# zfkuang/PaletteNeRF

Hardware: AMD Instinct MI355X
Metric: rendered_samples_per_sec (higher is better)
Workload: dtype f32 (field: f16x3 split products, fp32 accumulate); 1 GPU; configs[1]: NeRF-synthetic lego geometry (scene S0), -m nerf inference, 800x800, 1 view(s)/step, camera moving (one pose of the path per step); march_mode=native, fused_field=True, field_precision=f16x3, half_tables=False, ray_order=tile8, frames_in_flight=1, gathered_floats_per_ray=0, rccl_ranks=1, parallelism=single GPU

## Files before the change

### palettenerf_amd/csrc/frame.hip

```cpp
#include "pnr_common.hpp"
#include "march_core.hpp"
#include "grid_core.hpp"
#include "field_core.hpp"
#include "frame_plan.hpp"
#include <hip/hip_ext.h>
#include <vector>
#include <stdlib.h>

uint64_t pnr_internal_edit_device_bytes();
int pnr_internal_edit_upload(const pnr_palette_edit* edit, void* dst, hipStream_t s);
int pnr_internal_palette_field_forward(const pnr_palette_field_args* a, pnr_stream_t stream, int waves12);

#ifndef PNR_FRAME_LEVEL_PAIRS
#define PNR_FRAME_LEVEL_PAIRS 1
#endif
#ifndef PNR_FRAME_LEVEL_PAIRS_PAL
#define PNR_FRAME_LEVEL_PAIRS_PAL 0
#endif
namespace pnr {

struct FrameCtl {
    int32_t n_alive, n_step, step, done;
    int32_t iterations, pad0;
    unsigned long long rendered;
// ... 110 lines not shown
                                                                    float* __restrict__ depth, float* __restrict__ image, float* __restrict__ aux,
                                                                    FrameFinish fin) {
    if (fin.ctl && !fin.ctl->done) return;
    const uint32_t i = (blockIdx.x * kRayBlock + threadIdx.x) / LANES, q = threadIdx.x % LANES;
    if (i >= N) return;
    const uint32_t r = order ? (uint32_t)order[i] : i;
    if (q == 0) {
        const float d = sdepth[i];
        if (order) ws[r] = sws[i];
        if (fin.depth_raw) fin.depth_raw[r] = d;
        depth[r] = (fin.on & 2) ? finish_depth(fin, d, r) : d;
    }
    if (q < 3) { const float v = simage[(size_t)i * 3 + q]; image[(size_t)r * 3 + q] = (fin.on & 1) ? finish_channel(fin, v, sws[i], r, q) : v; }
    if (saux) {
        if (q * 4 < aux_stride) {
            float4 v = *reinterpret_cast<const float4*>(saux + (size_t)i * aux_stride + q * 4);
            if (q == 0 && (fin.on & 4)) {
                const float w = sws[i];
                v.x = finish_channel(fin, v.x, w, r, 0); v.y = finish_channel(fin, v.y, w, r, 1); v.z = finish_channel(fin, v.z, w, r, 2);
            }
            *reinterpret_cast<float4*>(aux + (size_t)r * aux_stride + q * 4) = v;
        }
    } else if (aux && (fin.on & 4) && q < 3) {
        aux[(size_t)r * aux_stride + q] = finish_channel(fin, aux[(size_t)r * aux_stride + q], sws[i], r, q);
    }
}

#ifdef PNR_MARCH_STATS
__device__ unsigned long long g_march_stats[8];
__device__ unsigned int g_march_max[64];
__device__ unsigned int g_march_hist[2][32];
__device__ unsigned int g_march_kinds[64][8];
#endif
__device__ __forceinline__ uint32_t shfl_xor_fresh(uint32_t v, int off) {
    int lane = (int)__builtin_amdgcn_mbcnt_hi(~0u, __builtin_amdgcn_mbcnt_lo(~0u, 0u));
    asm volatile("" : "+v"(lane));
    return (uint32_t)__builtin_amdgcn_ds_bpermute((lane ^ off) << 2, (int)v);
}
__device__ __forceinline__ unsigned long long shfl_xor_fresh(unsigned long long v, int off) {
    return ((unsigned long long)shfl_xor_fresh((uint32_t)(v >> 32), off) << 32) | shfl_xor_fresh((uint32_t)v, off);
}
__device__ __forceinline__ unsigned long long block_sum_u64(unsigned long long v, unsigned long long* sh ) {
    for (int off = PNR_WAVE / 2; off > 0; off >>= 1) v += shfl_xor_fresh(v, off);
    __syncthreads();
    if ((threadIdx.x & (PNR_WAVE - 1)) == 0) sh[threadIdx.x / PNR_WAVE] = v;
    __syncthreads();
    unsigned long long t = 0;
    for (int wv = 0; wv < (int)(kRayBlock / PNR_WAVE); wv++) t += sh[wv];
    return t;
}


#ifdef PNR_MARCH_TIMING
constexpr int kTimingWaves = 8192;
__device__ unsigned long long g_march_timing[kTimingWaves * 8];
__device__ int g_march_timing_iter = 3;
#define PNR_STAMP(k) do { if (timing && (threadIdx.x & 63) == 0) g_march_timing[(size_t)twave * 8 + (k)] = wall_clock64(); } while (0)
#else
#define PNR_STAMP(k) do { } while (0)
#endif
#ifndef PNR_MARCH_WAVES
#define PNR_MARCH_WAVES 4
#endif
#ifndef PNR_MARCH2_JUMPS
#define PNR_MARCH2_JUMPS true
#endif
#ifndef PNR_MARCH_WAVES_Q
#define PNR_MARCH_WAVES_Q 5
#endif
template <bool MIP, bool POW2, int MODE>
__global__ void __launch_bounds__(kRayBlock) __attribute__((amdgpu_waves_per_eu(MODE == 2 ? PNR_MARCH_WAVES_Q : PNR_MARCH_WAVES))) k_frame_march(const FrameCtl* __restrict__ prev, FrameCtl* __restrict__ cur, const int32_t* __restrict__ alive_prev,
                                                           int32_t* __restrict__ rays_alive, const int32_t* __restrict__ counts ,
                                                           int32_t* __restrict__ counts_cur ,
                                                           int32_t* __restrict__ scratch_rw, uint32_t N, uint32_t max_steps,
// ... 80 lines not shown
    const uint32_t* mip_lds = nullptr;
    if (mip_fast) {
        asm volatile("s_waitcnt vmcnt(0)" ::: "memory");
        __syncthreads();
        mip_lds = mip_smem;
    } else {
        mip_lds = stage_mip(mip, MIP ? p.mip_words : 0);
    }
    PNR_STAMP(2);
    uint32_t emitted = 0;
    uint32_t base = (uint32_t)(sums & 0xffffffffull), summed_to = blockIdx.x;
    for (uint32_t chunk = blockIdx.x; chunk < nchunks; chunk += gridDim.x) {
        if (threadIdx.x == 0) counts_cur[chunk] = 0;
        int index = index0;
        if (chunk != blockIdx.x) {
            unsigned long long pre = 0;
            for (uint32_t j = summed_to + threadIdx.x; j < chunk; j += kRayBlock) pre += (unsigned long long)counts[j];
            base += (uint32_t)block_sum_u64(pre, red);
            summed_to = chunk;
            const uint32_t slot = chunk * kRayBlock + threadIdx.x;
            index = slot < n_prev ? alive_prev[slot] : -1;
        }
        const int keep = index >= 0 ? 1 : 0;
        const unsigned long long alive_mask = __ballot(keep);
        if (lane == 0) csum[wave] = __popcll(alive_mask);
        __syncthreads();
        int woff = 0;
        for (int wv = 0; wv < wave; wv++) woff += csum[wv];
        __syncthreads();
        PNR_STAMP(3);
        uint32_t n = 0, step = 0;
        float t = 0.0f, far = -FLT_MAX, last_t = 0.0f;
        RayCtx c = {};
        if (keep) {
            n = base + (uint32_t)woff + (uint32_t)__popcll(alive_mask & ((1ull << lane) - 1ull));
            rays_alive[n] = index;
            ctx_init(c, rays_o + (size_t)index * 3, rays_d + (size_t)index * 3, p, grid, mip_lds);
            t = rays_t[index];
            const BoxHit bh = clip_to_box(c, fars[index]);
            far = bh.far;
            const float noise = (noises && prev->iterations == -1) ? noises[index] : 0.0f;
            t = fmaf(clampf(t * c.dt_gamma, c.dt_min, c.dt_max), noise, t);
            last_t = t;
            t = skip_to_box<MIP && POW2>(c, bh, t);
        }
        PNR_STAMP(4);
#ifdef PNR_MARCH_TIMING
        uint32_t my_probes = 0;
#endif
#ifdef PNR_MARCH_STATS
        unsigned long long probes = 0, empties = 0;
        unsigned int kinds[8] = {0, 0, 0, 0, 0, 0, 0, 0};
#endif
        bool active = keep && t < far;
        [[maybe_unused]] bool queued = false;
        [[maybe_unused]] uint32_t step_queued = 0;
        for (uint32_t round = 0;; round++) {
            const unsigned long long am = __ballot(active);
            if (am == 0ull) break;
            if constexpr (MODE == 1) { if (p.coop && __popcll(am) <= kCoopRays) break; }
            if constexpr (MODE == 2) {
                const bool give_up = active && round - step >= budget;
                const unsigned long long gm = __ballot(give_up);
                if (gm != 0ull) {
                    int32_t* qctr = qctr_all + ((prev->iterations + 1) & 1) * kQueueCtrs;
                    const int leader = __ffsll((long long)gm) - 1;
                    int slot0 = 0;
                    if (lane == leader) slot0 = atomicAdd(&qctr[0], __popcll(gm));
                    slot0 = __builtin_amdgcn_readlane(slot0, leader);
                    if (give_up) {
                        StragglerRec r;
                        r.n = (int32_t)n; r.index = index; r.step = (int32_t)step; r.t = t; r.last_t = last_t; r.far = far; r.pad0 = 0; r.pad1 = 0;
                        qrecs[(uint32_t)slot0 + (uint32_t)__popcll(gm & ((1ull << lane) - 1ull))] = r;
                        queued = true; step_queued = step; active = false;
                    }
                    if (gm == am) break;
                }
            }
// ... 663 lines not shown
    w.alive[1] = reinterpret_cast<int32_t*>(take(n * 4));
    w.rays_t = reinterpret_cast<float*>(take(n * 4));
    w.xyzs = reinterpret_cast<float*>(take(n * 12));
    w.dirs = reinterpret_cast<float*>(take(n * 12));
    w.deltas = reinterpret_cast<float*>(take(n * 8));
    w.enc = reinterpret_cast<float*>(take(n * 16 * 2 * 4));
    w.sigmas = reinterpret_cast<float*>(take(n * 4));
    w.rgbs = reinterpret_cast<float*>(take(n * 12));
    w.scratch = reinterpret_cast<int32_t*>(take((kHdr + 2 * (n / kRayBlock + 2)) * 4));
    w.partials[0] = reinterpret_cast<int32_t*>(take((kMaxMarchBlocks + kHostedBlocks) * 4));
    w.partials[1] = reinterpret_cast<int32_t*>(take((kMaxMarchBlocks + kHostedBlocks) * 4));
    w.enc_pal = w.enc_clip = w.aux = nullptr;
    w.edit = nullptr;
    if (aux_stride) {
        w.edit = take(pnr_internal_edit_device_bytes());
        w.enc_pal = reinterpret_cast<float*>(take(n * 16 * 2 * 4));
        if (with_clip) w.enc_clip = reinterpret_cast<float*>(take(n * 16 * 2 * 4));
        w.aux = reinterpret_cast<float*>(take(n * aux_stride * 4));
    }
    w.s_o = reinterpret_cast<float*>(take(n * 12)); w.s_d = reinterpret_cast<float*>(take(n * 12));
    w.s_noise = reinterpret_cast<float*>(take(n * 4)); w.s_far = reinterpret_cast<float*>(take(n * 4));
    w.s_ws = reinterpret_cast<float*>(take(n * 4)); w.s_depth = reinterpret_cast<float*>(take(n * 4));
    w.s_image = reinterpret_cast<float*>(take(n * 12));
    w.s_aux = aux_stride ? reinterpret_cast<float*>(take(n * aux_stride * 4)) : nullptr;
    w.hosted = reinterpret_cast<HostedConst*>(take(sizeof(HostedConst)));
    w.qctr = reinterpret_cast<int32_t*>(take(2 * kQueueCtrs * 4));
    w.qrecs = reinterpret_cast<StragglerRec*>(take(n * sizeof(StragglerRec)));
    w.rowflag = reinterpret_cast<uint8_t*>(take(n));
    w.bytes = off;
    return w;
}

struct FrameOpts {
    int aux_fusion, composite_fusion, hosted_tail, dynamic_tiles, march_budget, march_budget0, march_blocks, iteration_margin, block_skip, coop_march, palette_waves12;
};
static FrameOpts frame_opts_now() {
    return FrameOpts{g_opt_aux_fusion, g_opt_composite_fusion, g_opt_hosted_tail, g_opt_dynamic_tiles, g_opt_march_budget, g_opt_march_budget0, g_opt_march_blocks,
                     g_opt_iteration_margin, g_opt_block_skip, g_opt_coop_march, g_opt_palette_waves12};
}

using UnsortKernel = decltype(&k_frame_unsort_outputs<4>);
using MarchKernel = decltype(&k_frame_march<true, true, 1>);
using GridKernel = decltype(&k_frame_grid);
using FieldKernel = decltype(&k_frame_field<0, false>);

struct FramePlan {
    pnr_stream_t stream; const void* workspace;
    uint32_t N, max_steps, aux_stride, n_enc, march_lds;
    float T_thresh, density_scale, enc_scale;
    FrameWorkspace w;
    const float *in_o, *in_d, *in_far, *noise_p;
    float *out_ws, *out_depth, *out_image, *out_aux;
    const int32_t* ray_order;
    float *ray_ws, *ray_depth, *ray_image, *ray_aux;
    const uint8_t* bitfield; const uint32_t* mip; const float* packed_weights;
    bool with_clip, half_tables, hosted, use_mip, pow2, pal_composite_fused, timing, has_edit;
    int aux_fused;
    int composite_fused;
    MarchParams mp;
    GridArgs ga;
    pnr_palette_field_args pf;
    pnr_palette_edit edit;
    FrameFinish fin;
    FrameOpts opt;
    MarchKernel march, march_budgeted;
    GridKernel lookup; uint32_t lookup_y, lookup_z;
    FieldKernel field;
    uint64_t* stats; float* kernel_ms;
};
struct FrameProgress { int iter = 0; uint32_t alive_ub = 0, chunk = 0, looks = 0, prev_partials = 0; size_t ev_used = 0; };
struct PerDevice {
// ... 82 lines not shown
    ga.enc[0] = w.enc; ga.enc[1] = w.enc_pal; ga.enc[2] = w.enc_clip;
    p.lookup_y = 16; p.lookup_z = 1;
    if (p.half_tables && pal && p.with_clip) { p.lookup = k_frame_grid_h3; ga.table[0] = pal->embeddings_triple; }
    else if (p.half_tables && pal) { p.lookup = k_frame_grid_h2; ga.table[0] = pal->embeddings_pair; }
    else if (p.half_tables) { p.lookup = k_frame_grid_h1; ga.table[0] = a->embeddings; }
    else if (pal && p.with_clip && pal->embeddings_triple) { p.lookup = k_frame_grid_triple; ga.table[0] = pal->embeddings_triple; }
    else if (pal && !p.with_clip && pal->embeddings_pair) { p.lookup = k_frame_grid_pair; ga.table[0] = pal->embeddings_pair; p.lookup_y = PNR_FRAME_LEVEL_PAIRS_PAL ? 8 : 16; }
    else {
        p.lookup = k_frame_grid; p.lookup_y = PNR_FRAME_LEVEL_PAIRS == 2 ? 4 : (PNR_FRAME_LEVEL_PAIRS ? 8 : 16); p.lookup_z = p.n_enc;
        ga.table[0] = a->embeddings; ga.table[1] = pal ? pal->embeddings_palette : nullptr; ga.table[2] = p.with_clip ? pal->embeddings_clip : nullptr;
    }

    if (pal) {
        pnr_palette_field_args& pf = p.pf;
        pf.enc = w.enc; pf.enc_palette = w.enc_pal; pf.enc_clip = w.enc_clip; pf.level_stride = p.N; pf.dirs = w.dirs; pf.deltas = w.deltas;
        pf.packed = a->packed_weights; pf.num_basis = pal->num_basis;
        pf.clip_dim = pal->clip_dim; pf.pred_clip = pal->pred_clip; pf.density_scale = a->density_scale; pf.offsets_weight = pal->offsets_weight;
        pf.view_dep_weight = pal->view_dep_weight; pf.aux_stride = p.aux_stride; pf.sigmas = w.sigmas; pf.rgbs = w.rgbs; pf.aux = w.aux;
        pf.precision = a->field_precision; pf.xyzs = w.xyzs;
        for (int k = 0; k < 3; k++) pf.enc_scale[k] = a->enc_scale[k];
        pf.overflow_flag = a->watch_overflow ? w.scratch + 1 : nullptr;
        pf.tile_counter = opt.dynamic_tiles ? w.scratch + 2 : nullptr;
        if (p.aux_fused) { pf.weights_sum = p.out_ws; pf.aux_map = p.out_aux; pf.T_thresh = a->T_thresh; }
        if (p.pal_composite_fused) { pf.rays_t = w.rays_t; pf.weights_sum_rw = p.out_ws; pf.depth = p.out_depth; pf.image = p.out_image; }
        if (pal->edit && pal->edit->mode != 0) { p.has_edit = true; p.edit = *pal->edit; pf.edit_device = w.edit; }
    } else {
        p.enc_scale = a->enc_scale[0] > 0.0f ? a->enc_scale[0] : 1.0f;
        p.field = frame_field_kernel(a->field_precision, a->watch_overflow);
    }

    p.use_mip = a->mip && (a->H % 4) == 0 && pnr_occupancy_mip_bytes(a->C, a->H) <= 64 * 1024;
    p.pow2 = is_pow2f(a->bound) && (a->H & (a->H - 1)) == 0;
    p.mp = make_march_params(a->bound, a->dt_gamma, a->max_steps, a->C, a->H, p.use_mip);
    p.mp.block_skip = opt.block_skip ? 1u : 0u; p.mp.coop = opt.coop_march ? 1u : 0u;
    p.march_lds = p.mp.mip_words ? (2 * p.mp.mip_words + 8) * 4 : 0;
    p.hosted = opt.hosted_tail && p.use_mip && p.pow2 && p.mp.mip_words != 0 && (a->H % 64u) == 0;
    p.march = frame_march_kernel(p.use_mip, p.pow2, 1); p.march_budgeted = frame_march_kernel(true, true, 2);

    FrameFinish& fin = p.fin;
    fin.on = a->finish; fin.bg[0] = a->bg_color[0]; fin.bg[1] = a->bg_color[1]; fin.bg[2] = a->bg_color[2];
    fin.bg_map = a->bg_map; fin.nears = a->nears; fin.fars = a->fars;
    fin.depth_raw = a->depth_raw;
    return PNR_OK;
}

static int frame_begin(const pnr_nerf_frame_args* a, const FramePlan& p) {
    const FrameWorkspace& w = p.w;
    hipStream_t s = as_stream(p.stream);
    if (p.has_edit) {
        const int rc = pnr_internal_edit_upload(&p.edit, w.edit, s);
        if (rc != PNR_OK) return rc;
    }
    HostedConst hconst = {};
    hconst.qctr_all = w.qctr; hconst.qrecs = w.qrecs; hconst.rays_o = p.in_o; hconst.rays_d = p.in_d; hconst.bitfield = p.bitfield; hconst.mip = p.mip; hconst.p = p.mp;
    hconst.xyzs = w.xyzs; hconst.dirs = w.dirs; hconst.deltas = w.deltas; hconst.partials[0] = w.partials[0]; hconst.partials[1] = w.partials[1];
    FrameBegin fb = {};
    fb.order = a->ray_order; fb.rays_o = a->rays_o; fb.rays_d = a->rays_d; fb.nears_in = a->nears; fb.fars_in = a->fars;
    fb.aabb = a->aabb; fb.min_near = a->min_near; fb.nears_out = a->nears; fb.fars_out = a->fars;
    fb.so = w.s_o; fb.sd = w.s_d; fb.sf = w.s_far; fb.noises = a->noises; fb.snoise = w.s_noise;
    if (p.aux_stride) {
        if ((p.aux_stride & 3u) == 0 && (reinterpret_cast<uintptr_t>(p.out_aux) & 15u) == 0) { fb.aux_zero = p.out_aux; fb.aux_stride = p.aux_stride; }
        else if (hipMemsetAsync(p.out_aux, 0, (size_t)p.N * p.aux_stride * 4, s) != hipSuccess) return PNR_ERR_LAUNCH;
    }
    hipLaunchKernelGGL(k_frame_begin, dim3(cdiv(p.N, kRayBlock)), dim3(kRayBlock), 0, s, p.N, fb, w.alive[1], w.rays_t, p.out_ws, p.out_depth, p.out_image,
                       w.ctl, counts_of(p, 1), w.scratch, w.qctr, hconst, w.hosted);
    return PNR_OK;
}
// ... 213 lines not shown
```

### palettenerf_amd/csrc/march_core.hpp

```cpp
#pragma once
#include "pnr_common.hpp"
#include "lattice.hpp"
#include <float.h>
#include <string.h>
#include <stdlib.h>

namespace pnr {

__device__ __forceinline__ void near_far_of(float ox, float oy, float oz, float dx, float dy, float dz, const float* __restrict__ aabb, float min_near,
                                            float& near_out, float& far_out) {
    const float rdx = 1.0f / dx, rdy = 1.0f / dy, rdz = 1.0f / dz;
    float near = (aabb[0] - ox) * rdx, far = (aabb[3] - ox) * rdx, tmp;
    if (near > far) { tmp = near; near = far; far = tmp; }
    float ny = (aabb[1] - oy) * rdy, fy = (aabb[4] - oy) * rdy;
    if (ny > fy) { tmp = ny; ny = fy; fy = tmp; }
    if (near > fy || ny > far) { near_out = far_out = FLT_MAX; return; }
    if (ny > near) near = ny;
    if (fy < far) far = fy;
    float nz = (aabb[2] - oz) * rdz, fz = (aabb[5] - oz) * rdz;
    if (nz > fz) { tmp = nz; nz = fz; fz = tmp; }
    if (near > fz || nz > far) { near_out = far_out = FLT_MAX; return; }
    if (nz > near) near = nz;
    if (fz < far) far = fz;
    if (near < min_near) near = min_near;
    near_out = near;
    far_out = far;
}

struct RayCtx {
    float ox, oy, oz, dx, dy, dz, rdx, rdy, rdz;
    float bound, dt_gamma, dt_min, dt_max, rH, fC, fH, half_H;
    uint32_t H, H3;
    int maxlevel;
    const uint8_t* __restrict__ grid;
    const uint32_t* mip_any;
    const uint32_t* mip_all;
    const float* box;
    bool block_skip;
    mutable uint32_t cached_brick;
    mutable unsigned long long cached_bits;
    mutable uint32_t nojump_key;
#ifdef PNR_MARCH_TIMING
    mutable uint32_t n_loads;
#endif
};

struct MarchParams {
    float bound, dt_gamma, dt_min, dt_max;
    uint32_t C, H, max_steps;
    uint32_t mip_words;
    uint32_t block_skip;
    uint32_t coop;
};

static MarchParams make_march_params(float bound, float dt_gamma, uint32_t max_steps, uint32_t C, uint32_t H, bool with_mip) {
    MarchParams p;
    const float two_sqrt3 = 2.0f * 1.7320508075688772f;
    p.bound = bound; p.dt_gamma = dt_gamma;
    p.dt_min = two_sqrt3 / (float)max_steps;
    p.dt_max = two_sqrt3 * (float)(1 << (C - 1)) / (float)H;
    p.C = C; p.H = H; p.max_steps = max_steps;
    p.mip_words = with_mip ? (uint32_t)(((uint64_t)C * H * H * H / 64 + 31) / 32) : 0;
    p.block_skip = g_opt_block_skip ? 1u : 0u;
    p.coop = g_opt_coop_march ? 1u : 0u;
    return p;
}
static inline bool is_pow2f(float v) {
    uint32_t u; memcpy(&u, &v, 4);
    return v > 0.0f && (u & 0x7fffffu) == 0 && ((u >> 23) & 0xff) != 0 && ((u >> 23) & 0xff) != 0xff;
}

__device__ __forceinline__ void ctx_init(RayCtx& c, const float* __restrict__ o, const float* __restrict__ d, const MarchParams& p,
                                         const uint8_t* __restrict__ grid, const uint32_t* mip_lds) {
    c.ox = o[0]; c.oy = o[1]; c.oz = o[2];
    c.dx = d[0]; c.dy = d[1]; c.dz = d[2];
    c.rdx = 1.0f / c.dx; c.rdy = 1.0f / c.dy; c.rdz = 1.0f / c.dz;
    c.bound = p.bound; c.dt_gamma = p.dt_gamma; c.dt_min = p.dt_min; c.dt_max = p.dt_max;
    c.rH = 1.0f / (float)p.H; c.fC = (float)p.C; c.fH = (float)p.H; c.half_H = 0.5f * (float)p.H;
    c.H = p.H; c.H3 = p.H * p.H * p.H; c.maxlevel = (int)p.C - 1; c.grid = grid;
    c.mip_any = mip_lds;
    c.mip_all = mip_lds ? mip_lds + p.mip_words : nullptr;
    c.box = mip_lds ? reinterpret_cast<const float*>(mip_lds + 2 * p.mip_words) : nullptr;
    c.block_skip = mip_lds != nullptr && (p.H % 64u) == 0 && p.block_skip != 0;
    c.cached_brick = 0xffffffffu; c.cached_bits = 0ull;
    c.nojump_key = 0xffffffffu;
#ifdef PNR_MARCH_TIMING
    c.n_loads = 0;
#endif
}

struct BoxHit { float far, t_in, face, o, rd; bool entry_valid; };

__device__ __forceinline__ BoxHit clip_to_box(const RayCtx& c, float far) {
    BoxHit h; h.far = far; h.t_in = -FLT_MAX; h.face = 0.0f; h.o = 0.0f; h.rd = 0.0f; h.entry_valid = false;
    if (!c.box) return h;
    const float ax = (c.box[0] - c.ox) * c.rdx, bx = (c.box[3] - c.ox) * c.rdx;
    const float ay = (c.box[1] - c.oy) * c.rdy, by = (c.box[4] - c.oy) * c.rdy;
// ... 5 lines not shown
    if (t_in > t_out) { h.far = -FLT_MAX; return h; }
    h.far = fminf(far, fmaf(fabsf(t_out), 1e-5f, t_out));
    h.t_in = t_in; h.entry_valid = true;
    if (ex >= ey && ex >= ez) { h.face = ax <= bx ? c.box[0] : c.box[3]; h.o = c.ox; h.rd = c.rdx; }
    else if (ey >= ez)        { h.face = ay <= by ? c.box[1] : c.box[4]; h.o = c.oy; h.rd = c.rdy; }
    else                      { h.face = az <= bz ? c.box[2] : c.box[5]; h.o = c.oz; h.rd = c.rdz; }
    return h;
}
__device__ __forceinline__ float clip_far_to_box(const RayCtx& c, float far) { return clip_to_box(c, far).far; }

template <bool POW2>
__device__ __forceinline__ float skip_to_box(const RayCtx& c, const BoxHit& h, float t) {
    if constexpr (!POW2) return t;
    if (!h.entry_valid || !c.box || __float_as_uint(c.box[6]) != 1u) return t;
    if (!(h.t_in > t)) return t;
    const float cell = c.box[7];
    const float ard = fabsf(h.rd);
    if (!(ard < 1e6f)) return t;
    const float out = h.rd > 0.0f ? -cell : cell;
    const bool const_min = c.dt_gamma == 0.0f || (h.t_in + c.dt_max) * c.dt_gamma <= c.dt_min;
    const bool const_max = !const_min && t * c.dt_gamma >= c.dt_max;
    for (int k = 0; k < 8; k++) {
        const float plane = fmaf((float)k, out, h.face);
        const float b = (plane - h.o) * h.rd;
        const float eps = fmaf(c.bound * 2.3841858e-7f, ard, (fabsf(b) + 1.0f) * 9.5367432e-7f);
        if (!(b - t > 2.0f * eps)) return t;
        float q, prev;
        if (const_min) lattice_advance(t, fminf(c.dt_min, c.dt_max), b, q, prev);
        else if (const_max) lattice_advance(t, c.dt_max, b, q, prev);
        else lattice_walk(t, c.dt_gamma, c.dt_min, c.dt_max, b, q, prev);
        if (q - b > 2.0f * eps && b - prev > 2.0f * eps) return q;
    }
    return t;
}

__device__ __forceinline__ int level_of(float mx, int maxlevel) {
    const int e = (int)((__float_as_uint(mx) >> 23) & 0xffu) - 126;
    return min(maxlevel, max(0, e));
}

template <bool MIP>
__device__ __forceinline__ bool cell_occupied(const RayCtx& c, uint32_t index) {
    if constexpr (MIP) {
        const uint32_t brick = index >> 6, word = brick >> 5, bit = 1u << (brick & 31u);
        if (!(c.mip_any[word] & bit)) return false;
        if (c.mip_all[word] & bit) return true;
        if (brick != c.cached_brick) {
            c.cached_bits = *reinterpret_cast<const unsigned long long*>(c.grid + (size_t)brick * 8);
            c.cached_brick = brick;
#ifdef PNR_MARCH_TIMING
            c.n_loads++;
#endif
        }
        return (c.cached_bits >> (index & 63u)) & 1ull;
    }
    return c.grid[index >> 3] & (1u << (index & 7u));
}

__device__ __forceinline__ int empty_block_log2(const RayCtx& c, uint32_t index) {
    const uint32_t brick = index >> 6;
    const uint32_t lo = c.mip_any[(brick >> 6) * 2], hi = c.mip_any[(brick >> 6) * 2 + 1];
    if ((lo | hi) == 0) return 4;
    const uint32_t w = (brick & 32u) ? hi : lo;
    if (((w >> (brick & 24u)) & 0xffu) == 0) return 3;
    return ((w >> (brick & 31u)) & 1u) ? 0 : 2;
}
// ... 244 lines not shown
```

### palettenerf_amd/csrc/pnr_common.hpp

```cpp
#pragma once
#include <hip/hip_runtime.h>
#include <hip/hip_fp16.h>
#include <stdint.h>
#include "../../include/pnr.h"

#define PNR_WAVE 64

namespace pnr {

inline int check_launch() {
    hipError_t e = hipGetLastError();
    return e == hipSuccess ? PNR_OK : PNR_ERR_LAUNCH;
}
inline hipStream_t as_stream(pnr_stream_t s) { return reinterpret_cast<hipStream_t>(s); }
inline uint32_t cdiv(uint32_t a, uint32_t b) { return (a + b - 1) / b; }

constexpr int kMaxDevices = 64;
inline int current_device() { int d = 0; if (hipGetDevice(&d) != hipSuccess || d < 0 || d >= kMaxDevices) d = 0; return d; }
template <typename K>
inline bool ensure_dynamic_lds(K kernel, uint32_t bytes, bool* done ) {
    const int d = current_device();
    if (done[d]) return true;
    if (hipFuncSetAttribute(reinterpret_cast<const void*>(kernel), hipFuncAttributeMaxDynamicSharedMemorySize, (int)bytes) != hipSuccess) return false;
    done[d] = true;
// ... 38 lines not shown
typedef float f32x2 __attribute__((ext_vector_type(2)));
typedef float f32x4 __attribute__((ext_vector_type(4)));
template <typename T>
struct GlobalPtr { typedef const T __attribute__((address_space(1))) * type; };
template <typename T>
__device__ __forceinline__ void load8_fresh(const T* (&p)[8], T (&v)[8]) {
    asm volatile("" : "+v"(p[0]), "+v"(p[1]), "+v"(p[2]), "+v"(p[3]), "+v"(p[4]), "+v"(p[5]), "+v"(p[6]), "+v"(p[7]));
#pragma unroll
    for (int i = 0; i < 8; i++) v[i] = *(typename GlobalPtr<T>::type)(uintptr_t)p[i];
    __builtin_amdgcn_sched_barrier(0);
    asm volatile("" :: "v"(p[0]), "v"(p[1]), "v"(p[2]), "v"(p[3]), "v"(p[4]), "v"(p[5]), "v"(p[6]), "v"(p[7]));
}

__device__ __forceinline__ void lds_copy16(const void* gsrc, void* lds) {
    __builtin_amdgcn_global_load_lds((const __attribute__((address_space(1))) void*)gsrc, (__attribute__((address_space(3))) void*)lds, 16, 0, 0);
}
__device__ __forceinline__ void lds_copy_wait() { asm volatile("s_waitcnt vmcnt(0)" ::: "memory"); }
__device__ __forceinline__ uint32_t lds_address(const void* p) { return (uint32_t)reinterpret_cast<uintptr_t>(p); }

__device__ __forceinline__ int wave_inclusive_scan(int v) {
    const int lane = threadIdx.x & (PNR_WAVE - 1);
#pragma unroll
    for (int off = 1; off < PNR_WAVE; off <<= 1) {
        int n = __shfl_up(v, off, PNR_WAVE);
        if (lane >= off) v += n;
    }
    return v;
}

}

extern int g_opt_block_skip;
extern int g_opt_coop_march;
extern int g_opt_hosted_tail;
extern int g_opt_march_budget, g_opt_march_budget0;
extern int g_opt_march_blocks;
extern int g_opt_aux_fusion;
extern int g_opt_composite_fusion;
extern int g_opt_palette_waves12;
extern int g_opt_dynamic_tiles;
extern int g_opt_grid_fast;
extern int g_opt_train_coop;
extern int g_opt_mlp_f16x3;
extern int g_opt_coarse_image;
extern int g_opt_scatter_staged;
extern int g_opt_cell_merge;
extern int g_opt_grid_nt;
extern int g_opt_flex_coop;
extern int g_opt_iteration_margin;
```

### palettenerf_amd/csrc/raymarch.hip

```cpp
#include "pnr_common.hpp"
#include "march_core.hpp"
#include "sph_core.hpp"

namespace pnr {

constexpr uint32_t kBlock = 256;

__global__ void __launch_bounds__(256) k_build_mip(const unsigned long long* __restrict__ grid64, uint32_t nbricks, uint32_t words_per_mask,
                                                   uint32_t* __restrict__ mip) {
    const uint32_t b = blockIdx.x * blockDim.x + threadIdx.x;
    const unsigned long long w = b < nbricks ? grid64[b] : 0ull;
    const unsigned long long any = __ballot(w != 0ull), all = __ballot(b < nbricks && w == ~0ull);
    if ((threadIdx.x & 63) == 0) {
        const uint32_t word = b >> 5;
        if (word < words_per_mask) { mip[word] = (uint32_t)any; mip[words_per_mask + word] = (uint32_t)all; }
        if (word + 1 < words_per_mask) { mip[word + 1] = (uint32_t)(any >> 32); mip[words_per_mask + word + 1] = (uint32_t)(all >> 32); }
    }
}


__global__ void __launch_bounds__(kBlock) k_near_far(const float* __restrict__ rays_o, const float* __restrict__ rays_d,
                                                     const float* __restrict__ aabb, uint32_t N, float min_near,
                                                     float* __restrict__ nears, float* __restrict__ fars) {
    const uint32_t n = blockIdx.x * kBlock + threadIdx.x;
// ... 429 lines not shown
        if (to_srgb) x = x < 0.0031308f ? 12.92f * x : 1.055f * powf(x, 0.41666f) - 0.055f;
        b[k] = (uint8_t)(int)(x * 255.0f);
    }
    if (i0 + 3 < n && (reinterpret_cast<uintptr_t>(dst + i0) & 3u) == 0)
        *reinterpret_cast<uchar4*>(dst + i0) = make_uchar4(b[0], b[1], b[2], b[3]);
    else
        for (int k = 0; k < 4; k++) if (i0 + k < n) dst[i0 + k] = b[k];
}

__global__ void __launch_bounds__(kBlock) k_get_rays(const float* __restrict__ poses, uint32_t B, float fx, float fy, float cx, float cy, uint32_t W,
                                                     const long long* __restrict__ inds, uint32_t N, float* __restrict__ rays_o,
                                                     float* __restrict__ rays_d) {
    const uint32_t n = blockIdx.x * kBlock + threadIdx.x, b = blockIdx.y;
    if (n >= N) return;
    const uint32_t p = inds ? (uint32_t)inds[(size_t)b * N + n] : n;
    const float xs = (((float)(p % W) + 0.5f) - cx) / fx;
    const float ys = (((float)(p / W) + 0.5f) - cy) / fy;
    const float nrm = sqrtf(fmaf(xs, xs, fmaf(ys, ys, 1.0f)));
    const float d0 = xs / nrm, d1 = ys / nrm, d2 = 1.0f / nrm;
    const float* P = poses + (size_t)b * 16;
    float* o = rays_o + ((size_t)b * N + n) * 3;
    float* d = rays_d + ((size_t)b * N + n) * 3;
#pragma unroll
    for (int k = 0; k < 3; k++) {
        d[k] = fmaf(d2, P[k * 4 + 2], fmaf(d1, P[k * 4 + 1], d0 * P[k * 4 + 0]));
        o[k] = P[k * 4 + 3];
    }
}

}

int g_opt_block_skip = getenv("PNR_NO_BLOCK_SKIP") ? 0 : 1;
int g_opt_coop_march = getenv("PNR_NO_COOP_MARCH") ? 0 : 1;
int g_opt_hosted_tail = getenv("PNR_NO_HOSTED_TAIL") ? 0 : 1;
int g_opt_march_budget = getenv("PNR_MARCH_BUDGET") ? atoi(getenv("PNR_MARCH_BUDGET")) : 2;
int g_opt_march_budget0 = getenv("PNR_MARCH_BUDGET0") ? atoi(getenv("PNR_MARCH_BUDGET0")) : 0;
int g_opt_march_blocks = getenv("PNR_MARCH_BLOCKS") ? atoi(getenv("PNR_MARCH_BLOCKS")) : 0;
int g_opt_aux_fusion = getenv("PNR_NO_AUX_FUSION") ? 0 : 1;
int g_opt_composite_fusion = getenv("PNR_NO_COMPOSITE_FUSION") ? 0 : (getenv("PNR_COMPOSITE_FUSION") ? atoi(getenv("PNR_COMPOSITE_FUSION")) : 2);
int g_opt_iteration_margin = getenv("PNR_ITERATION_MARGIN") ? atoi(getenv("PNR_ITERATION_MARGIN")) : 0;
int g_opt_palette_waves12 = getenv("PNR_PALETTE_WAVES8") ? 0 : 1;
int g_opt_dynamic_tiles = getenv("PNR_DYNAMIC_TILES") ? 1 : 0;
int g_opt_grid_fast = getenv("PNR_NO_GRID_FAST") ? 0 : 1;
int g_opt_train_coop = getenv("PNR_NO_TRAIN_COOP") ? 0 : 1;
int g_opt_mlp_f16x3 = getenv("PNR_MLP_FP32") ? 0 : 1;
int g_opt_coarse_image = getenv("PNR_NO_COARSE_IMAGE") ? 0 : 1;
int g_opt_scatter_staged = getenv("PNR_NO_SCATTER_STAGED") ? 0 : 1;
int g_opt_cell_merge = getenv("PNR_NO_CELL_MERGE") ? 0 : 1;
int g_opt_flex_coop = getenv("PNR_NO_FLEX_COOP") ? 0 : 1;
int g_opt_grid_nt = getenv("PNR_GRID_NT") ? atoi(getenv("PNR_GRID_NT")) : 0;
int g_opt_adam_variant = 0;

using namespace pnr;

extern "C" {

int pnr_abi_version(void) { return 10; }

int pnr_set_option(const char* name, int value) {
    if (!name) return PNR_ERR_INVALID;
    if (!strcmp(name, "block_skip")) { g_opt_block_skip = value != 0; return PNR_OK; }
    if (!strcmp(name, "coop_march")) { g_opt_coop_march = value != 0; return PNR_OK; }
    if (!strcmp(name, "hosted_tail")) { g_opt_hosted_tail = value != 0; return PNR_OK; }
    if (!strcmp(name, "march_budget")) { g_opt_march_budget = value < 1 ? 1 : (value > 1024 ? 1024 : value); return PNR_OK; }
    if (!strcmp(name, "march_budget0")) { g_opt_march_budget0 = value < 0 ? 0 : (value > 1024 ? 1024 : value); return PNR_OK; }
    if (!strcmp(name, "march_blocks")) { g_opt_march_blocks = value < 0 ? 0 : value; return PNR_OK; }
    if (!strcmp(name, "aux_fusion")) { g_opt_aux_fusion = value != 0; return PNR_OK; }
    if (!strcmp(name, "composite_fusion")) { g_opt_composite_fusion = value < 0 ? 0 : (value > 2 ? 2 : value); return PNR_OK; }
    if (!strcmp(name, "palette_waves12")) { g_opt_palette_waves12 = value != 0; return PNR_OK; }
    if (!strcmp(name, "dynamic_tiles")) { g_opt_dynamic_tiles = value != 0; return PNR_OK; }
    if (!strcmp(name, "grid_fast")) { g_opt_grid_fast = value != 0; return PNR_OK; }
    if (!strcmp(name, "train_coop")) { g_opt_train_coop = value != 0; return PNR_OK; }
    if (!strcmp(name, "mlp_f16x3")) { g_opt_mlp_f16x3 = value != 0; return PNR_OK; }
    if (!strcmp(name, "coarse_image")) { g_opt_coarse_image = value != 0; return PNR_OK; }
    if (!strcmp(name, "cell_merge")) { g_opt_cell_merge = value != 0; return PNR_OK; }
    if (!strcmp(name, "scatter_staged")) { g_opt_scatter_staged = value != 0; return PNR_OK; }
    if (!strcmp(name, "flex_coop")) { g_opt_flex_coop = value != 0; return PNR_OK; }
    if (!strcmp(name, "grid_nt")) { g_opt_grid_nt = value & 3; return PNR_OK; }
    if (!strcmp(name, "adam_variant")) { g_opt_adam_variant = value & 7; return PNR_OK; }
    if (!strcmp(name, "iteration_margin")) { g_opt_iteration_margin = value < 0 ? 0 : (value > 64 ? 64 : value); return PNR_OK; }
    return PNR_ERR_INVALID;
}

const char* pnr_error_string(int code) {
    switch (code) {
        case PNR_OK: return "ok";
        case PNR_ERR_INVALID: return "invalid argument (null pointer or bad size)";
        case PNR_ERR_UNSUPPORTED: return "unsupported configuration";
        case PNR_ERR_LAUNCH: return "HIP kernel launch failed";
        case PNR_ERR_ALIGNMENT: return "an activation array does not start on a 16-byte boundary or holds fewer than four floats (pnr_mlp_* move tiles as 16-byte requests: copy such a view)";
        default: return "unknown error";
    }
}

int pnr_get_rays(const float* poses, uint32_t B, float fx, float fy, float cx, float cy, uint32_t H, uint32_t W, const int64_t* inds, uint32_t N,
// ... 199 lines not shown
```

Measured before the change: 3.064 billion samples/s.

## Add wave-level beam skip over empty space before ray marching

Adds a wave-cooperative beam test before marching begins on the first iteration. The wave bounds its rays' origins, directions and t-ranges, and each lane tests one slab of that beam against the mip occupancy bricks held in LDS. All rays then jump to the first slab that may be occupied, landed on their own step lattice. This is meant to cut the many empty-space probes at the start of each ray, at the cost of extra wave reductions and brick scans for every wave, including waves whose rays would have hit geometry early.

Measured after the change: 3.083 billion samples/s, median of 6. About the same (+0.6%).

```diff
diff --git a/palettenerf_amd/csrc/beam_core.hpp b/palettenerf_amd/csrc/beam_core.hpp
--- /dev/null
+++ b/palettenerf_amd/csrc/beam_core.hpp
@@ -0,0 +1,99 @@
+#pragma once
+#include "lattice.hpp"
+#include <float.h>
+
+namespace pnr {
+
+constexpr int kBeamSlabs = 64;
+constexpr int kBeamMaxBricks = 48;
+constexpr int kBeamLevels = 2;
+
+struct BeamBounds { float o_lo[3], o_hi[3], d_lo[3], d_hi[3], t_lo, t_hi; };
+struct BeamGrid { float bound, dt_gamma, dt_min, dt_max, half_H, slab; uint32_t H; int maxlevel; };
+
+PNR_HD float beam_slab_len(float bound, uint32_t H) { return 8.0f * fminf(1.0f, bound) / (float)H; }
+PNR_HD float beam_slab_start(const BeamBounds& b, float slab, int k) { return fmaf((float)k, slab, b.t_lo); }
+
+PNR_HD int beam_level_of(float mx, int maxlevel) {
+    const int e = (int)((lat_bits(mx) >> 23) & 0xffu) - 126;
+    return e < 0 ? 0 : (e > maxlevel ? maxlevel : e);
+}
+
+PNR_HD bool beam_slab_box(const BeamBounds& b, float t0, float t1, float lo[3], float hi[3]) {
+    bool ok = true;
+    for (int a = 0; a < 3; a++) {
+        const float p0 = b.d_lo[a] * t0, p1 = b.d_lo[a] * t1, p2 = b.d_hi[a] * t0, p3 = b.d_hi[a] * t1;
+        lo[a] = b.o_lo[a] + fminf(fminf(p0, p1), fminf(p2, p3));
+        hi[a] = b.o_hi[a] + fmaxf(fmaxf(p0, p1), fmaxf(p2, p3));
+        ok = ok && lo[a] - lo[a] == 0.0f && hi[a] - hi[a] == 0.0f && p0 == p0 && p1 == p1 && p2 == p2 && p3 == p3;
+    }
+    return ok;
+}
+
+PNR_HD void beam_level_bricks(const BeamGrid& g, int level, const float lo[3], const float hi[3], int blo[3], int bhi[3]) {
+    const float mip_bound = fminf(lat_float((uint32_t)(127 + level) << 23), g.bound);
+    const float rb = 1.0f / mip_bound;
+    const float top = (float)(g.H - 1);
+    for (int a = 0; a < 3; a++) {
+        const float fl = floorf(fmaf(lo[a], rb, 1.0f) * g.half_H) - 1.0f, fh = floorf(fmaf(hi[a], rb, 1.0f) * g.half_H) + 1.0f;
+        blo[a] = (int)fminf(top, fmaxf(0.0f, fl)) >> 2;
+        bhi[a] = (int)fminf(top, fmaxf(0.0f, fh)) >> 2;
+    }
+}
+
+PNR_HD void beam_slab_levels(const BeamGrid& g, const float lo[3], const float hi[3], float t0, float t1, int& l0, int& l1) {
+    const float w = 2.0f * fminf(1.0f, g.bound) / (float)g.H;
+    float nmin = 0.0f, nmax = 0.0f;
+    for (int a = 0; a < 3; a++) {
+        const float l = lo[a] - w, h = hi[a] + w;
+        nmin = fmaxf(nmin, l > 0.0f ? l : (h < 0.0f ? -h : 0.0f));
+        nmax = fmaxf(nmax, fmaxf(fabsf(l), fabsf(h)));
+    }
+    const float dlo = fminf(g.dt_max, fmaxf(g.dt_min, t0 * g.dt_gamma)) * 0.999f, dhi = fminf(g.dt_max, fmaxf(g.dt_min, t1 * g.dt_gamma)) * 1.001f;
+    const int p0 = beam_level_of(nmin, g.maxlevel), p1 = beam_level_of(nmax, g.maxlevel);
+    const int s0 = beam_level_of(dlo * g.half_H, g.maxlevel), s1 = beam_level_of(dhi * g.half_H, g.maxlevel);
+    l0 = p0 > s0 ? p0 : s0;
+    l1 = p1 > s1 ? p1 : s1;
+}
+
+template <class Test>
+PNR_HD bool beam_slab_full(const BeamGrid& g, const BeamBounds& b, int k, Test&& test) {
+    const float t0 = beam_slab_start(b, g.slab, k), t1 = beam_slab_start(b, g.slab, k + 1);
+    float lo[3], hi[3];
+    if (!beam_slab_box(b, t0, t1, lo, hi)) return true;
+    int l0, l1;
+    beam_slab_levels(g, lo, hi, t0, t1, l0, l1);
+    if (l1 - l0 >= kBeamLevels) return true;
+    for (int l = l0; l <= l1; l++) {
+        int blo[3], bhi[3];
+        beam_level_bricks(g, l, lo, hi, blo, bhi);
+        if ((bhi[0] - blo[0] + 1) * (bhi[1] - blo[1] + 1) * (bhi[2] - blo[2] + 1) > kBeamMaxBricks) return true;
+        if (test(l, blo, bhi)) return true;
+    }
+    return false;
+}
+
+PNR_HD float beam_land(float o, float d, float rd, float t, float t_safe, float bound, float cell , float dt_gamma, float dt_min, float dt_max) {
+    const float ard = fabsf(rd);
+    if (!(ard < 1e6f) || !(t_safe > t) || !(t_safe < 1e30f)) return t;
+    const float j = (fmaf(t_safe, d, o) + bound) / cell;
+    const float face = fmaf(d > 0.0f ? floorf(j) : ceilf(j), cell, -bound);
+    const float out = d > 0.0f ? -cell : cell;
+    const bool const_min = dt_gamma == 0.0f || (t_safe + dt_max) * dt_gamma <= dt_min;
+    const bool const_max = !const_min && t * dt_gamma >= dt_max;
+    for (int k = 0; k < 4; k++) {
+        const float plane = fmaf((float)k, out, face);
+        const float b = (plane - o) * rd;
+        const float eps = fmaf(bound * 2.3841858e-7f, ard, (fabsf(b) + 1.0f) * 9.5367432e-7f);
+        if (!(b <= t_safe)) continue;
+        if (!(b - t > 2.0f * eps)) return t;
+        float q, prev;
+        if (const_min) lattice_advance(t, fminf(dt_min, dt_max), b, q, prev);
+        else if (const_max) lattice_advance(t, dt_max, b, q, prev);
+        else lattice_walk(t, dt_gamma, dt_min, dt_max, b, q, prev);
+        if (q - b > 2.0f * eps && b - prev > 2.0f * eps) return q;
+    }
+    return t;
+}
+
+}
diff --git a/palettenerf_amd/csrc/frame.hip b/palettenerf_amd/csrc/frame.hip
--- a/palettenerf_amd/csrc/frame.hip
+++ b/palettenerf_amd/csrc/frame.hip
@@ -166,14 +166,6 @@
 __device__ unsigned int g_march_hist[2][32];
 __device__ unsigned int g_march_kinds[64][8];
 #endif
-__device__ __forceinline__ uint32_t shfl_xor_fresh(uint32_t v, int off) {
-    int lane = (int)__builtin_amdgcn_mbcnt_hi(~0u, __builtin_amdgcn_mbcnt_lo(~0u, 0u));
-    asm volatile("" : "+v"(lane));
-    return (uint32_t)__builtin_amdgcn_ds_bpermute((lane ^ off) << 2, (int)v);
-}
-__device__ __forceinline__ unsigned long long shfl_xor_fresh(unsigned long long v, int off) {
-    return ((unsigned long long)shfl_xor_fresh((uint32_t)(v >> 32), off) << 32) | shfl_xor_fresh((uint32_t)v, off);
-}
 __device__ __forceinline__ unsigned long long block_sum_u64(unsigned long long v, unsigned long long* sh ) {
     for (int off = PNR_WAVE / 2; off > 0; off >>= 1) v += shfl_xor_fresh(v, off);
     __syncthreads();
@@ -320,6 +312,7 @@
         uint32_t n = 0, step = 0;
         float t = 0.0f, far = -FLT_MAX, last_t = 0.0f;
         RayCtx c = {};
+        BoxHit bh0 = {};
         if (keep) {
             n = base + (uint32_t)woff + (uint32_t)__popcll(alive_mask & ((1ull << lane) - 1ull));
             rays_alive[n] = index;
@@ -330,8 +323,10 @@
             const float noise = (noises && prev->iterations == -1) ? noises[index] : 0.0f;
             t = fmaf(clampf(t * c.dt_gamma, c.dt_min, c.dt_max), noise, t);
             last_t = t;
-            t = skip_to_box<MIP && POW2>(c, bh, t);
-        }
+            bh0 = bh;
+        }
+        if constexpr (MODE == 1) { if (prev->iterations == -1) t = beam_skip<MIP, POW2>(c, p, mip_lds, bh0, keep != 0, t, far); }
+        if (keep) t = skip_to_box<MIP && POW2>(c, bh0, t);
         PNR_STAMP(4);
 #ifdef PNR_MARCH_TIMING
         uint32_t my_probes = 0;
@@ -1061,11 +1056,11 @@
 }
 
 struct FrameOpts {
-    int aux_fusion, composite_fusion, hosted_tail, dynamic_tiles, march_budget, march_budget0, march_blocks, iteration_margin, block_skip, coop_march, palette_waves12;
+    int aux_fusion, composite_fusion, hosted_tail, dynamic_tiles, march_budget, march_budget0, march_blocks, iteration_margin, block_skip, coop_march, palette_waves12, march_beam_skip;
 };
 static FrameOpts frame_opts_now() {
     return FrameOpts{g_opt_aux_fusion, g_opt_composite_fusion, g_opt_hosted_tail, g_opt_dynamic_tiles, g_opt_march_budget, g_opt_march_budget0, g_opt_march_blocks,
-                     g_opt_iteration_margin, g_opt_block_skip, g_opt_coop_march, g_opt_palette_waves12};
+                     g_opt_iteration_margin, g_opt_block_skip, g_opt_coop_march, g_opt_palette_waves12, g_opt_march_beam_skip};
 }
 
 using UnsortKernel = decltype(&k_frame_unsort_outputs<4>);
@@ -1214,7 +1209,7 @@
     p.use_mip = a->mip && (a->H % 4) == 0 && pnr_occupancy_mip_bytes(a->C, a->H) <= 64 * 1024;
     p.pow2 = is_pow2f(a->bound) && (a->H & (a->H - 1)) == 0;
     p.mp = make_march_params(a->bound, a->dt_gamma, a->max_steps, a->C, a->H, p.use_mip);
-    p.mp.block_skip = opt.block_skip ? 1u : 0u; p.mp.coop = opt.coop_march ? 1u : 0u;
+    p.mp.block_skip = opt.block_skip ? 1u : 0u; p.mp.coop = opt.coop_march ? 1u : 0u; p.mp.beam = opt.march_beam_skip ? 1u : 0u;
     p.march_lds = p.mp.mip_words ? (2 * p.mp.mip_words + 8) * 4 : 0;
     p.hosted = opt.hosted_tail && p.use_mip && p.pow2 && p.mp.mip_words != 0 && (a->H % 64u) == 0;
     p.march = frame_march_kernel(p.use_mip, p.pow2, 1); p.march_budgeted = frame_march_kernel(true, true, 2);
diff --git a/palettenerf_amd/csrc/march_core.hpp b/palettenerf_amd/csrc/march_core.hpp
--- a/palettenerf_amd/csrc/march_core.hpp
+++ b/palettenerf_amd/csrc/march_core.hpp
@@ -1,6 +1,7 @@
 #pragma once
 #include "pnr_common.hpp"
 #include "lattice.hpp"
+#include "beam_core.hpp"
 #include <float.h>
 #include <string.h>
 #include <stdlib.h>
@@ -51,6 +52,8 @@
     uint32_t mip_words;
     uint32_t block_skip;
     uint32_t coop;
+    uint32_t beam;
+    float beam_slab;
 };
 
 static MarchParams make_march_params(float bound, float dt_gamma, uint32_t max_steps, uint32_t C, uint32_t H, bool with_mip) {
@@ -63,6 +66,8 @@
     p.mip_words = with_mip ? (uint32_t)(((uint64_t)C * H * H * H / 64 + 31) / 32) : 0;
     p.block_skip = g_opt_block_skip ? 1u : 0u;
     p.coop = g_opt_coop_march ? 1u : 0u;
+    p.beam = g_opt_march_beam_skip ? 1u : 0u;
+    p.beam_slab = beam_slab_len(bound, H);
     return p;
 }
 static inline bool is_pow2f(float v) {
@@ -134,6 +139,78 @@
         if (q - b > 2.0f * eps && b - prev > 2.0f * eps) return q;
     }
     return t;
+}
+
+__device__ __forceinline__ uint32_t shfl_xor_fresh(uint32_t v, int off) {
+    int lane = (int)__builtin_amdgcn_mbcnt_hi(~0u, __builtin_amdgcn_mbcnt_lo(~0u, 0u));
+    asm volatile("" : "+v"(lane));
+    return (uint32_t)__builtin_amdgcn_ds_bpermute((lane ^ off) << 2, (int)v);
+}
+__device__ __forceinline__ unsigned long long shfl_xor_fresh(unsigned long long v, int off) {
+    return ((unsigned long long)shfl_xor_fresh((uint32_t)(v >> 32), off) << 32) | shfl_xor_fresh((uint32_t)v, off);
+}
+
+__device__ __forceinline__ float wave_min_f(float v) {
+    for (int off = PNR_WAVE / 2; off > 0; off >>= 1) v = fminf(v, __uint_as_float(shfl_xor_fresh(__float_as_uint(v), off)));
+    return v;
+}
+__device__ __forceinline__ float beam_safe_t(const MarchParams& p, const uint32_t* mip_lds, const BeamBounds& bb) {
+    const int lane = (int)(threadIdx.x & (PNR_WAVE - 1));
+    BeamGrid g;
+    g.bound = p.bound; g.dt_gamma = p.dt_gamma; g.dt_min = p.dt_min; g.dt_max = p.dt_max; g.half_H = 0.5f * (float)p.H; g.slab = p.beam_slab;
+    g.H = p.H; g.maxlevel = (int)p.C - 1;
+    bool full = false;
+    if (beam_slab_start(bb, g.slab, lane) < bb.t_hi) {
+        const uint32_t bricks_per_level = (p.H * p.H * p.H) >> 6;
+        full = beam_slab_full(g, bb, lane, [&](int level, const int* blo, const int* bhi) {
+            const uint32_t base = (uint32_t)level * bricks_per_level;
+            uint32_t any = 0;
+            for (int z = blo[2]; z <= bhi[2]; z++)
+                for (int y = blo[1]; y <= bhi[1]; y++) {
+                    const uint32_t myz = base + ((spread3((uint32_t)y) << 1) | (spread3((uint32_t)z) << 2));
+                    for (int x = blo[0]; x <= bhi[0]; x++) {
+                        const uint32_t brick = myz + spread3((uint32_t)x);
+                        any |= (mip_lds[brick >> 5] >> (brick & 31u)) & 1u;
+                    }
+                }
+            return any != 0;
+        });
+    }
+    const unsigned long long fm = __ballot(full);
+    if (fm != 0ull) return beam_slab_start(bb, g.slab, __ffsll((long long)fm) - 1);
+    const float t_end = beam_slab_start(bb, g.slab, kBeamSlabs);
+    return t_end < bb.t_hi ? t_end : FLT_MAX;
+}
+template <bool MIP, bool POW2>
+__device__ __forceinline__ float beam_skip(const RayCtx& c, const MarchParams& p, const uint32_t* mip_lds, const BoxHit& h, bool keep, float t, float far) {
+    if constexpr (!(MIP && POW2)) return t;
+    if (!p.beam || !mip_lds) return t;
+    const float* box = reinterpret_cast<const float*>(mip_lds + 2 * p.mip_words);
+    if (__float_as_uint(box[6]) != 1u) return t;
+    const bool marching = keep && t < far;
+    const float start = h.entry_valid ? fmaxf(t, h.t_in) : t;
+    const float mag = fmaxf(fmaxf(fmaxf(fabsf(c.ox), fabsf(c.oy)), fmaxf(fabsf(c.oz), fabsf(c.dx))), fmaxf(fmaxf(fabsf(c.dy), fabsf(c.dz)), fmaxf(fabsf(start), fabsf(far))));
+    const bool sane = mag < 1e30f;
+    const unsigned long long mm = __ballot(marching);
+    if (mm == 0ull || __ballot(marching && !sane) != 0ull) return t;
+    const bool has = marching;
+    BeamBounds bb;
+    bb.o_lo[0] = wave_min_f(has ? c.ox : FLT_MAX); bb.o_hi[0] = -wave_min_f(has ? -c.ox : FLT_MAX);
+    bb.o_lo[1] = wave_min_f(has ? c.oy : FLT_MAX); bb.o_hi[1] = -wave_min_f(has ? -c.oy : FLT_MAX);
+    bb.o_lo[2] = wave_min_f(has ? c.oz : FLT_MAX); bb.o_hi[2] = -wave_min_f(has ? -c.oz : FLT_MAX);
+    bb.d_lo[0] = wave_min_f(has ? c.dx : FLT_MAX); bb.d_hi[0] = -wave_min_f(has ? -c.dx : FLT_MAX);
+    bb.d_lo[1] = wave_min_f(has ? c.dy : FLT_MAX); bb.d_hi[1] = -wave_min_f(has ? -c.dy : FLT_MAX);
+    bb.d_lo[2] = wave_min_f(has ? c.dz : FLT_MAX); bb.d_hi[2] = -wave_min_f(has ? -c.dz : FLT_MAX);
+    bb.t_lo = wave_min_f(has ? start : FLT_MAX);
+    bb.t_hi = -wave_min_f(has ? -far : FLT_MAX);
+    const float t_safe = beam_safe_t(p, mip_lds, bb);
+    if (!has || !(t < t_safe)) return t;
+    if (far <= t_safe) return far;
+    const float adx = fabsf(c.dx), ady = fabsf(c.dy), adz = fabsf(c.dz);
+    float o = c.oz, d = c.dz, rd = c.rdz;
+    if (adx >= ady && adx >= adz) { o = c.ox; d = c.dx; rd = c.rdx; }
+    else if (ady >= adz) { o = c.oy; d = c.dy; rd = c.rdy; }
+    return beam_land(o, d, rd, t, t_safe, p.bound, box[7], p.dt_gamma, p.dt_min, p.dt_max);
 }
 
 __device__ __forceinline__ int level_of(float mx, int maxlevel) {
diff --git a/palettenerf_amd/csrc/pnr_common.hpp b/palettenerf_amd/csrc/pnr_common.hpp
--- a/palettenerf_amd/csrc/pnr_common.hpp
+++ b/palettenerf_amd/csrc/pnr_common.hpp
@@ -94,6 +94,7 @@
 
 extern int g_opt_block_skip;
 extern int g_opt_coop_march;
+extern int g_opt_march_beam_skip;
 extern int g_opt_hosted_tail;
 extern int g_opt_march_budget, g_opt_march_budget0;
 extern int g_opt_march_blocks;
diff --git a/palettenerf_amd/csrc/raymarch.hip b/palettenerf_amd/csrc/raymarch.hip
--- a/palettenerf_amd/csrc/raymarch.hip
+++ b/palettenerf_amd/csrc/raymarch.hip
@@ -485,6 +485,7 @@
 
 int g_opt_block_skip = getenv("PNR_NO_BLOCK_SKIP") ? 0 : 1;
 int g_opt_coop_march = getenv("PNR_NO_COOP_MARCH") ? 0 : 1;
+int g_opt_march_beam_skip = getenv("PNR_NO_BEAM_SKIP") ? 0 : 1;
 int g_opt_hosted_tail = getenv("PNR_NO_HOSTED_TAIL") ? 0 : 1;
 int g_opt_march_budget = getenv("PNR_MARCH_BUDGET") ? atoi(getenv("PNR_MARCH_BUDGET")) : 2;
 int g_opt_march_budget0 = getenv("PNR_MARCH_BUDGET0") ? atoi(getenv("PNR_MARCH_BUDGET0")) : 0;
@@ -514,6 +515,7 @@
     if (!name) return PNR_ERR_INVALID;
     if (!strcmp(name, "block_skip")) { g_opt_block_skip = value != 0; return PNR_OK; }
     if (!strcmp(name, "coop_march")) { g_opt_coop_march = value != 0; return PNR_OK; }
+    if (!strcmp(name, "march_beam_skip")) { g_opt_march_beam_skip = value != 0; return PNR_OK; }
     if (!strcmp(name, "hosted_tail")) { g_opt_hosted_tail = value != 0; return PNR_OK; }
     if (!strcmp(name, "march_budget")) { g_opt_march_budget = value < 1 ? 1 : (value > 1024 ? 1024 : value); return PNR_OK; }
     if (!strcmp(name, "march_budget0")) { g_opt_march_budget0 = value < 0 ? 0 : (value > 1024 ? 1024 : value); return PNR_OK; }
```
